# 17ai/eventql

Hardware: AMD Instinct MI355X
Metric: rows/sec scanned+aggregated, 1e9-row 4-col GROUP BY (higher is better)
Workload: dtype u64/f64; 1 GPU; config3; query=k, sum(v), count(1), sum(b) WHERE a>30000 AND b<30000 GROUP BY k, rows_per_gpu=1000000000, columns=4, encodings=UINT64_PLAIN/FLOAT_IEEE754, groups=1000, partitions=1, merge=none, groups_hint=given, float_sums=fast

## Files before the change

eventql_amd/csrc/codegen_kernels.inc:

```

namespace {

struct UpdWord {
  int word;
  int op;
  int tslot = -1;
  const char* constant = nullptr;
  bool narrow = false;
  int toff = -1;
};

struct Gen {
  const KernelPlan& kp;
  std::ostringstream s;
  const int NC, NW, S, W, SB;
  const bool grouped;
  std::vector<UpdWord> updw;

  explicit Gen(const KernelPlan& p)
      : kp(p), NC(int(p.cols.size())), NW(int(p.states.size())), S(p.lds_slots),
        W(p.words_per_slot()), SB(p.state_word_base()), grouped(p.key_mode != KEY_NONE) {
    for (const auto& a : kp.aggs) {
      switch (a.fn) {
        case EVQL_AGG_COUNT:
// ... 274 lines not shown
    for (int i = 0; i < NC; ++i) {
      if (only && !(*only)[i]) continue;
      s << ind << "u64 x" << i << "[EVQL_UNROLL][2]; u32 y" << i << "[EVQL_UNROLL][2];\n";
    }
    s << "#pragma unroll\n" << ind << "for (int u = 0; u < EVQL_UNROLL; ++u) {\n";
    s << ind << "  const u64 r = base + ((u64) (u * EVQL_BLOCK) + tid) * 2;\n";
    for (int i = 0; i < NC; ++i) {
      if (only && !(*only)[i]) continue;
      const ColAccess& c = kp.cols[i];
      switch (c.mode) {
        case ColAccess::PLAIN64:
          s << ind << "  evql_plain64_x2(A.col[" << i << "].base, A.col[" << i << "].pages, r, x" << i << "[u][0], x"
            << i << "[u][1]);\n";
          break;
        case ColAccess::PLAIN32:
          s << ind << "  evql_plain32_x2(A.col[" << i << "].base, A.col[" << i << "].pages, r, x" << i << "[u][0], x"
            << i << "[u][1]);\n";
          break;
        case ColAccess::BITPACKED:
          s << ind << "  evql_bitpacked_x2<" << c.bits << ">(A.col[" << i << "].base, A.col[" << i << "].pages, r, x"
            << i << "[u][0], x" << i << "[u][1]);\n";
          break;
        case ColAccess::NARROW:
          s << ind << "  evql_bitpacked_x2<" << c.bits << ">(A.col[" << i << "].base, r, x" << i
            << "[u][0], x" << i << "[u][1]);\n";
          break;
        case ColAccess::NARROW_F32:
          s << ind << "  evql_f32_x2(A.col[" << i << "].base, r, x" << i << "[u][0], x" << i
            << "[u][1]);\n";
          break;
        case ColAccess::SOA:
          s << ind << "  evql_soa_x2(A.col[" << i << "].soa, r, x" << i << "[u][0], x" << i
            << "[u][1]);\n";
          break;
      }
      if (c.has_tags) {
        s << ind << "  { const unsigned short tt = *reinterpret_cast<const unsigned short*>(A.col["
          << i << "].tags + r); y" << i << "[u][0] = tt & 0xffu; y" << i << "[u][1] = tt >> 8; }\n";
      } else {
        s << ind << "  y" << i << "[u][0] = 0; y" << i << "[u][1] = 0;\n";
      }
    }
    s << ind << "}\n";
  }

  bool prunes() const { return !kp.zone_conjuncts.empty(); }
  bool zone_test = false;
  template <typename Loop>
  void tile_loop_twice(const char* ind, Loop emit_loop) {
    zone_test = false;
    if (!prunes()) {
      emit_loop();
      return;
    }
    s << ind << "if (!A.tile_skip) {\n";
    emit_loop();
    s << ind << "} else {\n";
    zone_test = true;
    emit_loop();
    zone_test = false;
    s << ind << "}\n";
  }
  void zone_skip(const char* ind, const char* on_skip, bool count = true) {
    if (!zone_test) return;
    const uint64_t T = uint64_t(kp.tile_rows());
    const uint64_t zones = T >= kZoneRows ? T / kZoneRows : 1;
    s << ind << "{\n";
    if (T >= kZoneRows) {
      s << ind << "  const u64 zi = (A.tile0 + t) * " << zones << "ull;\n";
    } else {
      s << ind << "  const u64 zi = ((A.tile0 + t) * (u64) EVQL_TILE_ROWS) / EVQL_ZONE_ROWS;\n";
    }
    s << ind << "  if (evql_zones_excluded<" << zones << ">(A.tile_skip, zi)) { " << on_skip
      << (count ? " ++zskipped;" : "") << " continue; }\n";
    s << ind << "}\n";
  }
  void zone_skip_decl(const char* ind) {
    if (prunes()) s << ind << "u32 zskipped = 0;  // tiles this workgroup skipped\n";
  }
  void zone_skip_flush(const char* ind) {
    if (prunes()) s << ind << "if (tid == 0 && zskipped) atomicAdd(&A.counters[5], (u64) zskipped);\n";
  }

  void eval_call(const char* ind, int j, const std::vector<bool>* only = nullptr) {
    s << ind << "evql_eval_row(A, r + " << j << ", (r + " << j << " >= A.row_begin) && (r + " << j
      << " < A.row_end)";
    for (int i = 0; i < NC; ++i) {
      if (only && !(*only)[i]) {
        s << ", 0ull, 0u";
        continue;
      }
      s << ", x" << i << "[u][" << j << "], y" << i << "[u][" << j << "]";
    }
    s << ", o);\n";
  }

  void scan_kernel() {
    s << "struct EvqlAcc {\n  u64 passed;\n  u64 spilled;\n";
    if (!grouped) s << "  u64 w[" << (NW > 0 ? NW : 1) << "];\n";
    if (!grouped && kp.need_first_row) s << "  u64 first;\n";
    if (grouped && S > 0) {
      s << "  int cs[EVQL_LCACHE];\n  u64 cfirst[EVQL_LCACHE];\n  u64 cw[EVQL_LCACHE][EVQL_NUPD];\n"
           "  u32 cv;\n";
    }
    s << "};\n\n";
    if (grouped && S > 0) {
      s << "template <int J>\n";
      s << "__device__ __forceinline__ void evql_flush_entry(u64* lds, EvqlAcc& acc) {\n";
      s << "  const int cs = acc.cs[J];\n";
      if (kp.need_first_row) {
        s << "  evql_atomic<EVQL_OP_MIN_U64>(&" << lds_word(kp.first_row_word(), "cs") << ", acc.cfirst[J]);\n";
        s << "  acc.cfirst[J] = 0xFFFFFFFFFFFFFFFFull;\n";
      }
      for (int i = 0; i < U(); ++i) {
        s << "  evql_atomic<" << op_name(updw[i].op) << ">(&" << lds_word(SB + updw[i].word, "cs")
          << ", acc.cw[J][" << i << "]);\n";
        s << "  acc.cw[J][" << i << "] = evql_op_identity<" << op_name(updw[i].op) << ">();\n";
      }
      s << "}\n";
      s << "__device__ __forceinline__ void evql_flush_private(u64* lds, EvqlAcc& acc) {\n";
      for (int j = 0; j < kp.lane_cache; ++j) {
        s << "  if (acc.cs[" << j << "] >= 0) { evql_flush_entry<" << j << ">(lds, acc); acc.cs[" << j
          << "] = -1; }\n";
      }
      s << "}\n\n";
    }

    s << "__device__ __forceinline__ void evql_update(const EvqlArgs& A, u64* lds, EvqlAcc& acc,\n"
         "                                            const bool bypass, const u64 row, "
         "const EvqlRowOut& o) {\n";
    s << "  acc.passed += o.live ? 1 : 0;\n";
    if (!grouped) {
      if (kp.need_first_row) s << "  if (o.live && row < acc.first) acc.first = row;\n";
      for (int i = 0; i < U(); ++i) {
        s << "  if (o.uc[" << i << "]) acc.w[" << updw[i].word << "] = evql_combine<"
          << op_name(updw[i].op) << ">(acc.w[" << updw[i].word << "], o.ub[" << i << "]);\n";
      }
      s << "}\n\n";
    } else {
      auto updates = [&](bool global, const char* slot, const char* ind) {
        if (kp.need_first_row) {
          s << ind << "evql_atomic<EVQL_OP_MIN_U64>(&"
            << (global ? gtab_word(kp.first_row_word(), slot) : lds_word(kp.first_row_word(), slot))
            << ", row);\n";
        }
        for (int i = 0; i < U(); ++i) {
          s << ind << "if (o.uc[" << i << "]) evql_atomic<" << op_name(updw[i].op) << ">(&"
            << (global ? gtab_word(SB + updw[i].word, slot) : lds_word(SB + updw[i].word, slot))
            << ", o.ub[" << i << "]);\n";
        }
      };
      if (S > 0) {
        s << "  int s = -1;\n";
        s << "  if (o.live && !bypass) {\n";
        s << "    if (o.knull) { s = EVQL_LDS_SLOTS + 1; lds[s] = 0; }\n";
        s << "    else if (o.ident == EVQL_EMPTY) { s = EVQL_LDS_SLOTS; lds[s] = 0; }\n";
        if (kp.has_ident2()) {
          s << "    else s = evql_lds_find2<16>(lds, lds + EVQL_LSTRIDE, EVQL_LDS_SLOTS - 1, o.ident, "
               "o.ident2, (u32) evql_mix64(o.ident));\n";
        } else {
          s << "    else s = evql_lds_find<16>(lds, EVQL_LDS_SLOTS - 1, o.ident, (u32) "
               "evql_mix64(o.ident));\n";
        }
        s << "    if (s < 0) atomicAdd(reinterpret_cast<u32*>(&lds[EVQL_WORDS * EVQL_LSTRIDE]), 1u);\n";
        s << "  }\n";
        s << "  if (s >= 0) {\n";
        s << "    bool hit = false;\n";
        for (int j = 0; j < kp.lane_cache; ++j) {
          s << "    {\n      const bool h = acc.cs[" << j << "] == s;\n      hit = hit || h;\n";
          if (kp.need_first_row) {
            s << "      acc.cfirst[" << j << "] = (h && row < acc.cfirst[" << j << "]) ? row : acc.cfirst["
              << j << "];\n";
          }
          for (int i = 0; i < U(); ++i) {
            s << "      if (h && o.uc[" << i << "]) acc.cw[" << j << "][" << i << "] = evql_combine<"
              << op_name(updw[i].op) << ">(acc.cw[" << j << "][" << i << "], o.ub[" << i << "]);\n";
          }
          s << "    }\n";
        }
        s << "    if (!hit) {\n";
        for (int j = 0; j < kp.lane_cache; ++j) {
          s << "      {\n        const bool v = acc.cv == " << j << "u;\n";
          s << "        if (v && acc.cs[" << j << "] >= 0) evql_flush_entry<" << j << ">(lds, acc);\n";
          s << "        acc.cs[" << j << "] = v ? s : acc.cs[" << j << "];\n";
          if (kp.need_first_row) {
            s << "        acc.cfirst[" << j << "] = v ? row : acc.cfirst[" << j << "];\n";
          }
          for (int i = 0; i < U(); ++i) {
            s << "        acc.cw[" << j << "][" << i << "] = (v && o.uc[" << i << "]) ? o.ub[" << i
              << "] : acc.cw[" << j << "][" << i << "];\n";
          }
          s << "      }\n";
        }
        if (kp.lane_cache > 1) {
          s << "      acc.cv = (acc.cv + 1u) & " << (kp.lane_cache - 1) << "u;\n";
        }
        s << "    }\n  }\n";
        s << "  const bool spill = o.live && s < 0;\n";
        s << "  acc.spilled += spill ? 1 : 0;\n";
      } else {
        s << "  const bool spill = o.live;\n";
      }
      s << "  if (spill) {\n";
      s << "    i64 gs;\n";
      s << "    if (o.knull) { gs = (i64) A.gcap + 1; A.gtab[(u64) gs * EVQL_WORDS] = 0; }\n";
      s << "    else if (o.ident == EVQL_EMPTY) { gs = (i64) A.gcap; A.gtab[(u64) gs * EVQL_WORDS] = 0; }\n";
      if (kp.has_ident2()) {
        s << "    else gs = evql_gtab_find2(A.gtab, EVQL_WORDS, A.gcap, o.ident, o.ident2, "
             "evql_mix64(o.ident));\n";
      } else {
        s << "    else gs = evql_gtab_find(A.gtab, EVQL_WORDS, A.gcap, o.ident, evql_mix64(o.ident));\n";
      }
      s << "    if (gs < 0) { atomicOr(&A.status[0], EVQL_ST_TABLE_FULL); }\n";
      s << "    else {\n";
      updates(true, "gs", "      ");
      s << "    }\n  }\n}\n\n";
    }

    if (grouped && S > 0) {
      s << "__device__ __forceinline__ void evql_lds_init(u64* lds) {\n";
      s << "  if (threadIdx.x == 0) lds[EVQL_WORDS * EVQL_LSTRIDE] = 0;\n";
      s << "  for (u32 i = threadIdx.x; i < EVQL_LSTRIDE; i += blockDim.x) {\n";
      s << "    lds[i] = EVQL_EMPTY;\n";
      if (kp.has_ident2()) s << "    lds[1 * EVQL_LSTRIDE + i] = EVQL_EMPTY;\n";
      if (kp.need_first_row) {
        s << "    " << lds_word(kp.first_row_word(), "i") << " = 0xFFFFFFFFFFFFFFFFull;\n";
      }
      for (int w = 0; w < NW; ++w) {
        s << "    " << lds_word(SB + w, "i") << " = evql_op_identity<" << op_name(kp.states[w].op)
          << ">();\n";
      }
      s << "  }\n}\n\n";
      s << "template <bool EXCL>\n";
      s << "__device__ __forceinline__ void evql_lds_flush(const EvqlArgs& A, u64* lds) {\n";
      s << "  const bool excl = EXCL && evql_lds_peek32(reinterpret_cast<const u32*>(&lds[EVQL_WORDS * EVQL_LSTRIDE])) "
           "== 0;\n";
      s << "  for (u32 s = threadIdx.x; s < EVQL_LSTRIDE; s += blockDim.x) {\n";
      s << "    const u64 k = lds[s];\n    if (k == EVQL_EMPTY) continue;\n";
      s << "    i64 gs;\n";
      s << "    if (s == EVQL_LDS_SLOTS) gs = (i64) A.gcap;\n";
      s << "    else if (s == EVQL_LDS_SLOTS + 1) gs = (i64) A.gcap + 1;\n";
      if (kp.has_ident2()) {
        s << "    else gs = evql_gtab_find2(A.gtab, EVQL_WORDS, A.gcap, k, lds[EVQL_LSTRIDE + s], "
             "evql_mix64(k));\n";
      } else {
        s << "    else gs = evql_gtab_find(A.gtab, EVQL_WORDS, A.gcap, k, evql_mix64(k));\n";
      }
      s << "    if (gs < 0) { atomicOr(&A.status[0], EVQL_ST_TABLE_FULL); continue; }\n";
      s << "    if (s >= EVQL_LDS_SLOTS) A.gtab[(u64) gs * EVQL_WORDS] = 0;\n";
      s << "    if (excl) {\n";
      if (kp.need_first_row) {
        s << "      " << gtab_word(kp.first_row_word(), "gs") << " = " << lds_word(kp.first_row_word(), "s")
          << ";\n";
      }
      for (int w = 0; w < NW; ++w) {
        s << "      " << gtab_word(SB + w, "gs") << " = " << lds_word(SB + w, "s") << ";\n";
      }
      s << "      continue;\n    }\n";
      if (kp.need_first_row) {
        s << "    evql_atomic<EVQL_OP_MIN_U64>(&" << gtab_word(kp.first_row_word(), "gs") << ", "
          << lds_word(kp.first_row_word(), "s") << ");\n";
      }
      for (int w = 0; w < NW; ++w) {
        s << "    evql_atomic<" << op_name(kp.states[w].op) << ">(&" << gtab_word(SB + w, "gs") << ", "
          << lds_word(SB + w, "s") << ");\n";
      }
      s << "  }\n}\n\n";
    }

    s << "extern \"C\" __global__ void __launch_bounds__(EVQL_BLOCK) evql_scan_agg(const EvqlArgs A) {\n";
    s << "  const u32 tid = threadIdx.x;\n";
    if (grouped && S > 0) {
      s << "  __shared__ u64 lds[EVQL_WORDS * EVQL_LSTRIDE + 1];\n";
      s << "  evql_lds_init(lds);\n  __syncthreads();\n";
    } else {
      s << "  u64* lds = nullptr;\n";
    }
    s << "  EvqlAcc acc;\n  acc.passed = 0;\n  acc.spilled = 0;\n";
    if (grouped && S > 0) {
      s << "  acc.cv = 0;\n";
      for (int j = 0; j < kp.lane_cache; ++j) {
        s << "  acc.cs[" << j << "] = -1;\n  acc.cfirst[" << j << "] = 0xFFFFFFFFFFFFFFFFull;\n";
        for (int i = 0; i < U(); ++i) {
          s << "  acc.cw[" << j << "][" << i << "] = evql_op_identity<" << op_name(updw[i].op) << ">();\n";
        }
      }
    }
    if (!grouped) {
      for (int w = 0; w < NW; ++w) {
        s << "  acc.w[" << w << "] = evql_op_identity<" << op_name(kp.states[w].op) << ">();\n";
      }
      if (kp.need_first_row) s << "  acc.first = 0xFFFFFFFFFFFFFFFFull;\n";
    }
    zone_skip_decl("  ");
    tile_loop_twice("  ", [&] {
    s << "  u32 tile_no = 0;\n";
    s << "  for (u64 t = blockIdx.x; t < A.ntiles; t += gridDim.x, ++tile_no) {\n";
    zone_skip("    ", "");
    if (grouped) {
      s << "    if ((tile_no & 15u) == 0 && (__hip_atomic_load(&A.status[0], __ATOMIC_RELAXED, "
           "__HIP_MEMORY_SCOPE_AGENT) & EVQL_ST_TABLE_FULL)) break;\n";
    }
    if (grouped && S > 0) {
      s << "    const bool bypass = evql_lds_peek32(reinterpret_cast<const u32*>(&lds[EVQL_WORDS * EVQL_LSTRIDE])) "
           ">= 4u * EVQL_BLOCK;\n";
    } else {
      s << "    const bool bypass = false;\n";
    }
    s << "    const u64 base = (A.tile0 + t) * (u64) EVQL_TILE_ROWS;\n";
    tile_loads("    ");
    s << "#pragma unroll\n    for (int u = 0; u < EVQL_UNROLL; ++u) {\n";
    s << "      const u64 r = base + ((u64) (u * EVQL_BLOCK) + tid) * 2;\n";
    s << "      EvqlRowOut o;\n";
    for (int j = 0; j < 2; ++j) {
      eval_call("      ", j);
      s << "      evql_update(A, lds, acc, bypass, r + " << j << ", o);\n";
    }
    s << "    }\n  }\n";
    });

    zone_skip_flush("  ");
    s << "  {\n    const u64 p = evql_wave_reduce<EVQL_OP_ADD_U64>(acc.passed);\n";
    s << "    if ((tid & 63u) == 0 && p) atomicAdd(&A.counters[0], p);\n";
    s << "    const u64 sp = evql_wave_reduce<EVQL_OP_ADD_U64>(acc.spilled);\n";
    s << "    if ((tid & 63u) == 0 && sp) atomicAdd(&A.counters[1], sp);\n  }\n";
    if (!grouped) {
      s << "  __shared__ u64 red[(EVQL_BLOCK / 64) * " << (NW + 1) << "];\n";
      s << "  const u32 wave = tid >> 6;\n";
      for (int w = 0; w < NW; ++w) {
        s << "  { const u64 v = evql_wave_reduce<" << op_name(kp.states[w].op) << ">(acc.w[" << w
          << "]); if ((tid & 63u) == 0) red[wave * " << (NW + 1) << " + " << w << "] = v; }\n";
      }
      s << "  { const u64 v = evql_wave_reduce<EVQL_OP_ADD_U64>(acc.passed); if ((tid & 63u) == 0) "
           "red[wave * "
        << (NW + 1) << " + " << NW << "] = v; }\n";
      if (kp.need_first_row) {
        s << "  { const u64 v = evql_wave_reduce<EVQL_OP_MIN_U64>(acc.first); if ((tid & 63u) == 0 && "
             "v != 0xFFFFFFFFFFFFFFFFull) evql_atomic<EVQL_OP_MIN_U64>(&A.gtab["
          << kp.first_row_word() << "], v); }\n";
      }
      s << "  __syncthreads();\n";
      s << "  if (tid == 0) {\n";
      s << "    u64 any = 0;\n";
      s << "    for (u32 k = 0; k < EVQL_BLOCK / 64; ++k) any += red[k * " << (NW + 1) << " + " << NW
        << "];\n";
      s << "    if (any) {\n      A.gtab[0] = 0;\n";
      for (int w = 0; w < NW; ++w) {
        s << "      { u64 v = red[" << w << "]; for (u32 k = 1; k < EVQL_BLOCK / 64; ++k) v = evql_combine<"
          << op_name(kp.states[w].op) << ">(v, red[k * " << (NW + 1) << " + " << w
          << "]); evql_atomic<" << op_name(kp.states[w].op) << ">(&A.gtab[" << (SB + w)
          << "], v); }\n";
      }
      s << "    }\n  }\n";
    } else if (S > 0) {
      s << "  evql_flush_private(lds, acc);\n";
      s << "  __syncthreads();\n";
      s << "  evql_lds_flush<false>(A, lds);\n";
    }
    s << "}\n\n";
  }

  void bare_scan_kernels() {
    const int NOUT = int(kp.scan_out.size());
    std::vector<bool> where_cols(size_t(NC), false);
    if (kp.where) {
      std::vector<uint32_t> used;
      expr_inputs(kp.where, &used);
      for (uint32_t u : used) {
        if (u < uint32_t(NC)) where_cols[u] = true;
      }
    }
    int n_nullable = 0;
    for (int k = 0; k < NOUT; ++k) n_nullable += kp.scan_out_nullable[k] ? 1 : 0;
    const int stage_steps =
        uint64_t(kp.tile_rows()) * uint64_t(8 * NOUT + n_nullable) <= 48 * 1024 ? kp.unroll : 1;
    s << "#define EVQL_NOUT " << NOUT << "\n";
    s << "#define EVQL_NWAVE (EVQL_BLOCK / 64)\n";
    s << "#define EVQL_STAGE_STEPS " << stage_steps << "\n";
    s << "#define EVQL_STAGE_ROWS (EVQL_STAGE_STEPS * EVQL_BLOCK * 2)\n";
    s << "static_assert(EVQL_UNROLL * EVQL_NWAVE <= 64, \"one wave scans the wave totals of a tile\");\n";
    s << "struct EvqlScanArgs {\n"
         "  const u64* tile_offset;  // [ntiles + 1]: passing rows in front of tile t of the scan\n"
         "  u64 t0, t1;              // the window: tiles [t0, t1)\n"
         "  u64 window_base;         // tile_offset[t0]\n"
         "  u64 window_rows;         // tile_offset[t1] - window_base: rows of every output array\n"
         "  u64* words;              // [EVQL_NOUT][window_rows]\n"
         "  u8* tags;                // [EVQL_NOUT][window_rows], written for nullable outputs only\n"
         "};\n\n";
    row_function(n_literals, [&](Emitter& em) {
      s << "__device__ __forceinline__ void evql_scan_select(const EvqlArgs& A, const u64 row";
      for (int i = 0; i < NC; ++i) s << ", const u64 r" << i << ", const u32 g" << i;
      s << ", u64 (&w)[EVQL_NOUT], u32 (&q)[EVQL_NOUT]) {\n";
      col_decls();
      em.ind = "  ";
      for (int k = 0; k < NOUT; ++k) {
        const ExprPtr& e = kp.scan_out[k];
        if (e->kind == Expr::INPUT && e->type == EVQL_T_STRING) {
          s << "  w[" << k << "] = A.col[" << e->input << "].strpos[row]; q[" << k << "] = g" << e->input
            << ";\n";
          continue;
        }
        Val v = em.emit(e);
        s << em.o.str();
        em.o.str("");
        s << "  w[" << k << "] = " << Emitter::as_bits(v) << "; q[" << k << "] = " << v.g << ";\n";
      }
      s << "}\n\n";
    });
    s << "__device__ __forceinline__ void evql_run_store(u64* out, const u64 at, const u64 cap, const u64* src, "
         "u32 n) {\n"
         "  typedef u64 evql_u64x2 __attribute__((ext_vector_type(2)));\n"
         "  if (at >= cap) return;\n"
         "  if ((u64) n > cap - at) n = (u32) (cap - at);\n"
         "  u64* const dst = out + at;\n"
         "  const u32 head = (n > 0 && ((u64) dst & 8ull)) ? 1u : 0u;\n"
         "  const u32 pairs = (n - head) >> 1;\n"
         "  if (threadIdx.x == 0 && head) dst[0] = src[0];\n"
         "  for (u32 i = threadIdx.x; i < pairs; i += EVQL_BLOCK) {\n"
         "    evql_u64x2 v;\n    v.x = src[head + 2 * i];\n    v.y = src[head + 2 * i + 1];\n"
         "    *reinterpret_cast<evql_u64x2*>(dst + head + 2 * i) = v;\n  }\n"
         "  if (threadIdx.x == 0 && ((n - head) & 1u)) dst[n - 1] = src[n - 1];\n"
         "}\n\n";

    s << "extern \"C\" __global__ void __launch_bounds__(EVQL_BLOCK) evql_scan_count(const EvqlArgs A, "
         "u32* tile_count) {\n";
    s << "  const u32 tid = threadIdx.x;\n";
    s << "  __shared__ u32 wsum[EVQL_NWAVE];\n";
    zone_skip_decl("  ");
    tile_loop_twice("  ", [&] {
    s << "  for (u64 t = blockIdx.x; t < A.ntiles; t += gridDim.x) {\n";
    zone_skip("    ", "if (tid == 0) tile_count[t] = 0;");
    s << "    const u64 base = (A.tile0 + t) * (u64) EVQL_TILE_ROWS;\n";
    tile_loads("    ", &where_cols);
    s << "    u32 cnt = 0;\n";
    s << "#pragma unroll\n    for (int u = 0; u < EVQL_UNROLL; ++u) {\n";
    s << "      const u64 r = base + ((u64) (u * EVQL_BLOCK) + tid) * 2;\n";
    s << "      EvqlRowOut o;\n";
    for (int j = 0; j < 2; ++j) {
      eval_call("      ", j, &where_cols);
      s << "      cnt += (u32) __popcll(__ballot(o.live));\n";
    }
    s << "    }\n";
    s << "    if ((tid & 63u) == 0) wsum[tid >> 6] = cnt;\n";
    s << "    __syncthreads();\n";
    s << "    if (tid == 0) {\n      u32 total = 0;\n";
    s << "      for (u32 k = 0; k < EVQL_NWAVE; ++k) total += wsum[k];\n";
    s << "      tile_count[t] = total;\n    }\n";
    s << "    __syncthreads();\n";
    s << "  }\n";
    });
    zone_skip_flush("  ");
    s << "}\n\n";

    s << "extern \"C\" __global__ void __launch_bounds__(EVQL_BLOCK) evql_scan_emit(const EvqlArgs A, "
         "const EvqlScanArgs S) {\n";
    s << "  const u32 tid = threadIdx.x, lane = tid & 63u, wave = tid >> 6;\n";
    s << "  __shared__ u64 sw[EVQL_NOUT * EVQL_STAGE_ROWS];\n";
    if (n_nullable) s << "  __shared__ u8 sq[" << n_nullable << " * EVQL_STAGE_ROWS];\n";
    s << "  __shared__ u32 wpre[EVQL_UNROLL * EVQL_NWAVE + 1];\n";
    s << "  for (u64 t = S.t0 + blockIdx.x; t < S.t1; t += gridDim.x) {\n";
    s << "    const u64 dst0 = S.tile_offset[t] - S.window_base;\n";
    s << "    if (S.tile_offset[t + 1] == S.tile_offset[t]) continue;\n";
    s << "    const u64 base = (A.tile0 + t) * (u64) EVQL_TILE_ROWS;\n";
    tile_loads("    ");
    s << "    u32 live = 0;  // bit 2u + j: row (u, j) of this lane passes\n";
    s << "#pragma unroll\n    for (int u = 0; u < EVQL_UNROLL; ++u) {\n";
    s << "      const u64 r = base + ((u64) (u * EVQL_BLOCK) + tid) * 2;\n";
    s << "      EvqlRowOut o;\n";
    s << "      u32 wcnt = 0;\n";
    for (int j = 0; j < 2; ++j) {
      eval_call("      ", j);
      s << "      live |= o.live ? (1u << (2 * u + " << j << ")) : 0u;\n";
      s << "      wcnt += (u32) __popcll(__ballot(o.live));\n";
    }
    s << "      if (lane == 0) wpre[u * EVQL_NWAVE + wave] = wcnt;\n";
    s << "    }\n    __syncthreads();\n";
    s << "    if (wave == 0) {\n";
    s << "      const u32 v = lane < EVQL_UNROLL * EVQL_NWAVE ? wpre[lane] : 0u;\n";
    s << "      u32 incl = v;\n";
    s << "#pragma unroll\n      for (int d = 1; d < 64; d <<= 1) { const u32 x = __shfl_up(incl, d, 64); "
         "if ((int) lane >= d) incl += x; }\n";
    s << "      if (lane < EVQL_UNROLL * EVQL_NWAVE) wpre[lane] = incl - v;\n";
    s << "      if (lane == EVQL_UNROLL * EVQL_NWAVE - 1) wpre[EVQL_UNROLL * EVQL_NWAVE] = incl;\n";
    s << "    }\n    __syncthreads();\n";
    s << "#pragma unroll\n    for (int u0 = 0; u0 < EVQL_UNROLL; u0 += EVQL_STAGE_STEPS) {\n";
    s << "      const u32 g0 = wpre[u0 * EVQL_NWAVE], g1 = wpre[(u0 + EVQL_STAGE_STEPS) * EVQL_NWAVE];\n";
    s << "#pragma unroll\n      for (int u = u0; u < u0 + EVQL_STAGE_STEPS; ++u) {\n";
    s << "        const u64 r = base + ((u64) (u * EVQL_BLOCK) + tid) * 2;\n";
    s << "        const bool l0 = (live >> (2 * u)) & 1u, l1 = (live >> (2 * u + 1)) & 1u;\n";
    s << "        const u64 b0 = __ballot(l0), b1 = __ballot(l1);\n";
    s << "        u32 rank = wpre[u * EVQL_NWAVE + wave] - g0;\n";
    s << "        rank = __builtin_amdgcn_mbcnt_hi((u32) (b0 >> 32), __builtin_amdgcn_mbcnt_lo((u32) b0, rank));\n";
    s << "        rank = __builtin_amdgcn_mbcnt_hi((u32) (b1 >> 32), __builtin_amdgcn_mbcnt_lo((u32) b1, rank));\n";
    for (int j = 0; j < 2; ++j) {
      s << "        if (l" << j << ") {\n";
      s << "          u64 w[EVQL_NOUT]; u32 q[EVQL_NOUT];\n";
      s << "          evql_scan_select(A, r + " << j;
      for (int i = 0; i < NC; ++i) s << ", x" << i << "[u][" << j << "], y" << i << "[u][" << j << "]";
      s << ", w, q);\n";
      int nk = 0;
      for (int k = 0; k < NOUT; ++k) {
        s << "          sw[" << k << " * EVQL_STAGE_ROWS + rank] = w[" << k << "];\n";
        if (kp.scan_out_nullable[k]) {
          s << "          sq[" << nk++ << " * EVQL_STAGE_ROWS + rank] = (u8) (q[" << k << "] & 1u);\n";
        }
      }
      s << "          rank += 1;\n        }\n";
    }
    s << "      }\n      __syncthreads();\n";
    s << "      const u32 n = g1 - g0;\n";
    s << "      const u64 at = dst0 + g0;\n";
    {
      int nk = 0;
      for (int k = 0; k < NOUT; ++k) {
        s << "      evql_run_store(S.words + " << k << " * S.window_rows, at, S.window_rows, sw + " << k
          << " * EVQL_STAGE_ROWS, n);\n";
        if (kp.scan_out_nullable[k]) {
          s << "      for (u32 i = tid; i < n && at + i < S.window_rows; i += EVQL_BLOCK) S.tags[" << k
            << " * S.window_rows + at + i] = sq[" << nk++ << " * EVQL_STAGE_ROWS + i];\n";
        }
      }
    }
    s << "      __syncthreads();\n";
    s << "    }\n  }\n}\n\n";
  }

  void where_rows_kernel() {
    s << "extern \"C\" __global__ void __launch_bounds__(EVQL_BLOCK) evql_where_rows(const EvqlArgs A, "
         "u8* acc) {\n";
    s << "  const u32 tid = threadIdx.x;\n";
    s << "  for (u64 t = blockIdx.x; t < A.ntiles; t += gridDim.x) {\n";
    s << "    const u64 base = (A.tile0 + t) * (u64) EVQL_TILE_ROWS;\n";
    tile_loads("    ");
    s << "#pragma unroll\n    for (int u = 0; u < EVQL_UNROLL; ++u) {\n";
    s << "      const u64 r = base + ((u64) (u * EVQL_BLOCK) + tid) * 2;\n";
    s << "      EvqlRowOut o;\n";
    for (int j = 0; j < 2; ++j) {
      eval_call("      ", j);
      s << "      if (r + " << j << " < A.row_end) acc[r + " << j << "] = o.live ? 1 : 0;\n";
    }
    s << "    }\n  }\n}\n\n";
  }

  void partition_kernels() {
    const int frw = kp.first_row_word();
    s << "#define EVQL_PBITS " << kp.part_bits << "\n#define EVQL_NPART " << (1 << kp.part_bits)
      << "\n";
    s << "__device__ __forceinline__ u32 evql_bucket(u64 ident) { return (u32) (evql_mix64(ident ^ "
         "0x5851f42d4c957f2dull) >> (64 - EVQL_PBITS)); }\n\n";
    const int cbits = kp.part_bits <= 8 ? kp.part_bits : 6;
    const int fbits = kp.part_bits - cbits;
    s << "#define EVQL_CBITS " << cbits << "\n#define EVQL_FBITS " << fbits << "\n";
    s << "#define EVQL_NCOARSE " << (1 << cbits) << "\n#define EVQL_NFINE " << (1 << fbits) << "\n";
    s << "struct EvqlPartArgs {\n  u64 tiles_per_wg;\n  u32* counts;      // [bucket][workgroup]\n"
         "  const u64* bucket_start;  // [NPART + 1] tuple index\n  u64* tuples;\n  u64 nwg;\n"
         "  u64* tuples_tmp;  // coarse-bucket order (two-level only)\n"
         "  u32* cursors;     // [NCOARSE] + [NPART] reservation cursors, zeroed per launch\n"
         "  u64* dense;       // dense group records [kind, identity, ...] of the buckets\n"
         "  u64 dense_cap;    // ... whose groups all fitted the LDS table (records)\n"
         "  u64 coarse_cap;   // fused form: capacity (tuples) of every coarse bucket of tuples_tmp\n};\n\n";
    const bool fused = kp.part_fused && fbits > 0;
    s << "#define EVQL_ST_PART_OVERFLOW 64u\n";
    if (fused) {
      s << "#define EVQL_CSTART(c_) ((u64) (c_) * P.coarse_cap)\n";
      s << "#define EVQL_CEND(c_) ((u64) (c_) * P.coarse_cap + ((u64) P.cursors[c_] < P.coarse_cap ? "
           "(u64) P.cursors[c_] : P.coarse_cap))\n";
    } else {
      s << "#define EVQL_CSTART(c_) (P.bucket_start[(u64) (c_) << EVQL_FBITS])\n";
      s << "#define EVQL_CEND(c_) (P.bucket_start[(u64) ((c_) + 1) << EVQL_FBITS])\n";
    }
    s << "__device__ __forceinline__ void evql_tuple_store(u32* p, const u32* v) {\n"
         "#pragma unroll\n"
         "  for (int x = 0; x < EVQL_TUPLE_U32; x += (EVQL_TUPLE_U32 % 4 == 0 ? 4 : 2)) {\n"
         "    if (EVQL_TUPLE_U32 % 4 == 0) *reinterpret_cast<uint4*>(p + x) = make_uint4(v[x], v[x + 1], "
         "v[x + 2], v[x + 3]);\n"
         "    else *reinterpret_cast<uint2*>(p + x) = make_uint2(v[x], v[x + 1]);\n  }\n}\n";
    s << "__device__ __forceinline__ void evql_tuple_load(const u32* p, u32* v) {\n"
         "#pragma unroll\n"
         "  for (int x = 0; x < EVQL_TUPLE_U32; x += (EVQL_TUPLE_U32 % 4 == 0 ? 4 : 2)) {\n"
         "    if (EVQL_TUPLE_U32 % 4 == 0) { const uint4 t = *reinterpret_cast<const uint4*>(p + x); "
         "v[x] = t.x; v[x + 1] = t.y; v[x + 2] = t.z; v[x + 3] = t.w; }\n"
         "    else { const uint2 t = *reinterpret_cast<const uint2*>(p + x); v[x] = t.x; v[x + 1] = "
         "t.y; }\n  }\n}\n\n";

    if (!fused) {
    s << "extern \"C\" __global__ void __launch_bounds__(EVQL_BLOCK) evql_part_count(const EvqlArgs A, "
         "const EvqlPartArgs P) {\n";
    s << "  const u32 tid = threadIdx.x;\n";
    s << "  __shared__ u32 hist[EVQL_NPART];\n";
    s << "  for (u32 i = tid; i < EVQL_NPART; i += EVQL_BLOCK) hist[i] = 0;\n  __syncthreads();\n";
    s << "  const u64 t0 = (u64) blockIdx.x * P.tiles_per_wg;\n";
    s << "  const u64 t1 = t0 + P.tiles_per_wg < A.ntiles ? t0 + P.tiles_per_wg : A.ntiles;\n";
    tile_loop_twice("  ", [&] {
    s << "  for (u64 t = t0; t < t1; ++t) {\n";
    zone_skip("    ", "", false);
    s << "    const u64 base = (A.tile0 + t) * (u64) EVQL_TILE_ROWS;\n";
    tile_loads("    ");
    s << "#pragma unroll\n    for (int u = 0; u < EVQL_UNROLL; ++u) {\n";
    s << "      const u64 r = base + ((u64) (u * EVQL_BLOCK) + tid) * 2;\n";
    s << "      EvqlRowOut o;\n";
    for (int j = 0; j < 2; ++j) {
      eval_call("      ", j);
      s << "      if (o.live) atomicAdd(&hist[evql_bucket(o.ident)], 1u);\n";
    }
    s << "    }\n  }\n";
    });
    s << "  __syncthreads();\n";
    s << "  for (u32 i = tid; i < EVQL_NPART; i += EVQL_BLOCK) P.counts[(u64) i * P.nwg + blockIdx.x] = "
         "hist[i];\n";
    s << "}\n\n";
    }

    s << "extern \"C\" __global__ void __launch_bounds__(EVQL_BLOCK) evql_part_scatter(const EvqlArgs A, "
         "const EvqlPartArgs P) {\n";
    s << "  const u32 tid = threadIdx.x;\n";
    s << "  __shared__ u32 hist[EVQL_NCOARSE];\n";
    s << "  __shared__ u64 gbase[EVQL_NCOARSE];\n";
    if (fused) {
      s << "  __shared__ u32 fhist[EVQL_NPART];\n";
      s << "  for (u32 i = tid; i < EVQL_NPART; i += EVQL_BLOCK) fhist[i] = 0;\n";
    }
    s << "  u32* const dst = reinterpret_cast<u32*>(EVQL_FBITS ? P.tuples_tmp : P.tuples);\n";
    s << "  u64 passed = 0;\n";
    s << "  const u64 t0 = (u64) blockIdx.x * P.tiles_per_wg;\n";
    s << "  const u64 t1 = t0 + P.tiles_per_wg < A.ntiles ? t0 + P.tiles_per_wg : A.ntiles;\n";
    zone_skip_decl("  ");
    tile_loop_twice("  ", [&] {
    s << "  for (u64 t = t0; t < t1; ++t) {\n";
    zone_skip("    ", "");
    s << "    const u64 base = (A.tile0 + t) * (u64) EVQL_TILE_ROWS;\n";
    tile_loads("    ");
    s << "    for (u32 i = tid; i < EVQL_NCOARSE; i += EVQL_BLOCK) hist[i] = 0;\n";
    s << "    __syncthreads();\n";
    s << "#pragma unroll\n    for (int u = 0; u < EVQL_UNROLL; ++u) {\n";
    s << "      const u64 r = base + ((u64) (u * EVQL_BLOCK) + tid) * 2;\n";
    s << "      EvqlRowOut o;\n";
    for (int j = 0; j < 2; ++j) {
      eval_call("      ", j);
      s << "      if (o.live) atomicAdd(&hist[evql_bucket(o.ident) >> EVQL_FBITS], 1u);\n";
    }
    s << "    }\n    __syncthreads();\n";
    s << "    for (u32 i = tid; i < EVQL_NCOARSE; i += EVQL_BLOCK) {\n";
    s << "      const u32 c = hist[i];\n";
    if (fused) {
      s << "      u64 gb = EVQL_EMPTY;\n";
      s << "      if (c) {\n";
      s << "        const u64 at = (u64) atomicAdd(&P.cursors[i], c);\n";
      s << "        if (at + c <= P.coarse_cap) gb = (u64) i * P.coarse_cap + at;\n";
      s << "        else atomicOr(&A.status[0], EVQL_ST_PART_OVERFLOW);\n";
      s << "      }\n";
      s << "      gbase[i] = gb;\n";
    } else {
      s << "      gbase[i] = P.bucket_start[(u64) i << EVQL_FBITS] + (c ? (u64) atomicAdd(&P.cursors[i], c) "
           ": 0ull);\n";
    }
    s << "      hist[i] = 0;\n    }\n    __syncthreads();\n";
    s << "#pragma unroll\n    for (int u = 0; u < EVQL_UNROLL; ++u) {\n";
    s << "      const u64 r = base + ((u64) (u * EVQL_BLOCK) + tid) * 2;\n";
    s << "      EvqlRowOut o;\n";
    for (int j = 0; j < 2; ++j) {
      eval_call("      ", j);
      s << "      if (o.live) {\n";
      s << "        passed += 1;\n";
      if (fused) {
        s << "        const u32 fb = evql_bucket(o.ident);\n";
        s << "        const u32 b = fb >> EVQL_FBITS;\n";
        s << "        atomicAdd(&fhist[fb], 1u);\n";
      } else {
        s << "        const u32 b = evql_bucket(o.ident) >> EVQL_FBITS;\n";
      }
      s << "        const u64 pos = gbase[b] + atomicAdd(&hist[b], 1u);\n";
      s << "        u32 tv[EVQL_TUPLE_U32];\n";
      s << "        tv[EVQL_TUPLE_U32 - 1] = 0;\n";
      tuple_put("        ", off_ident, kp.narrow_ident, "o.ident");
      if (kp.has_ident2()) tuple_put("        ", off_ident2, false, "o.ident2");
      if (kp.need_first_row) {
        tuple_put("        ", off_row, kp.narrow_first_row, "r + " + std::to_string(j));
      }
      for (int i = 0; i < U(); ++i) {
        if (updw[i].tslot < 0) continue;
        tuple_put("        ", updw[i].toff, updw[i].narrow, "o.ub[" + std::to_string(i) + "]");
      }
      if (fused) {
        s << "        if (gbase[b] != EVQL_EMPTY) evql_tuple_store(dst + pos * EVQL_TUPLE_U32, tv);\n";
      } else {
        s << "        evql_tuple_store(dst + pos * EVQL_TUPLE_U32, tv);\n";
      }
      s << "      }\n";
    }
    s << "    }\n    __syncthreads();\n  }\n";
    });
    if (fused) {
      s << "  __syncthreads();\n";
      s << "  for (u32 i = tid; i < EVQL_NPART; i += EVQL_BLOCK) {\n";
      s << "    const u32 c = fhist[i];\n";
      s << "    if (c) atomicAdd(const_cast<u64*>(&P.bucket_start[i]), (u64) c);\n  }\n";
    }
    zone_skip_flush("  ");
    s << "  { const u64 p = evql_wave_reduce<EVQL_OP_ADD_U64>(passed);\n";
    s << "    if ((tid & 63u) == 0 && p) atomicAdd(&A.counters[0], p); }\n";
    s << "}\n\n";

    if (fbits > 0) {
      const int TWn = tuple_u32;
      const int rtif = TWn <= 4 ? 4 : (TWn <= 8 ? 2 : 1);
      s << "#define EVQL_RTIF " << rtif << "\n";
      s << "extern \"C\" __global__ void __launch_bounds__(EVQL_BLOCK) evql_part_refine(const EvqlArgs "
           "A, const EvqlPartArgs P) {\n";
      s << "  const u32 tid = threadIdx.x;\n";
      if (fused) {
        s << "  if (__hip_atomic_load(&A.status[0], __ATOMIC_RELAXED, __HIP_MEMORY_SCOPE_AGENT) & "
             "EVQL_ST_PART_OVERFLOW) return;\n";
      }
// ... 211 lines not shown
```

eventql_amd/csrc/evql_device.h:

```cpp
#ifndef EVQL_DEVICE_H
#define EVQL_DEVICE_H

typedef unsigned long long u64;
typedef long long i64;
typedef unsigned int u32;
typedef unsigned char u8;

#define EVQL_EMPTY 0xFFFFFFFFFFFFFFFFull
#define EVQL_MAX_COLS 16
#define EVQL_MAX_LITS 32
#define EVQL_WAVE 64

#define EVQL_ST_DIV_BY_ZERO 1u
#define EVQL_ST_TABLE_FULL 2u
#define EVQL_ST_MOD_BY_ZERO 4u

struct EvqlColArg {
  const u64* pages;
  const u64* soa;
  const u8* tags;
  u64 npages;
  const u64* strpos;
  const u8* base;
};
// ... 243 lines not shown
  return true;
}
__device__ __forceinline__ bool evql_str_affix(const EvqlStr& s, const EvqlStr& affix, bool at_end) {
  if (s.len < affix.len) return false;
  const u32 off = at_end ? s.len - affix.len : 0;
  for (u32 i = 0; i < affix.len; ++i) {
    if (evql_str_byte(s, off + i) != evql_str_byte(affix, i)) return false;
  }
  return true;
}
__device__ __forceinline__ int evql_str_cmp(const EvqlStr& a, const EvqlStr& b) {
  const u32 n = a.len < b.len ? a.len : b.len;
  for (u32 i = 0; i < n; ++i) {
    const u32 x = evql_str_byte(a, i), y = evql_str_byte(b, i);
    if (x != y) return x < y ? -1 : 1;
    if (x == 0) break;
  }
  return a.len < b.len ? -1 : (a.len > b.len ? 1 : 0);
}

__device__ __forceinline__ double evql_as_f64(u64 v) { return __longlong_as_double((i64) v); }
__device__ __forceinline__ u64 evql_f64_bits(double v) { return (u64) __double_as_longlong(v); }

#define EVQL_OP_ADD_U64 0
#define EVQL_OP_ADD_F64 1
#define EVQL_OP_MIN_U64 2
#define EVQL_OP_MAX_U64 3
#define EVQL_OP_MIN_I64 4
#define EVQL_OP_MAX_I64 5
#define EVQL_OP_MIN_F64 6
#define EVQL_OP_MAX_F64 7

template <int OP>
__device__ __forceinline__ u64 evql_op_identity() {
  switch (OP) {
    case EVQL_OP_MIN_U64: return 0xFFFFFFFFFFFFFFFFull;
    case EVQL_OP_MAX_U64: return 0ull;
    case EVQL_OP_MIN_I64: return 0x7FFFFFFFFFFFFFFFull;
    case EVQL_OP_MAX_I64: return 0x8000000000000000ull;
    case EVQL_OP_MIN_F64: return 0x7FF0000000000000ull;
    case EVQL_OP_MAX_F64: return 0xFFF0000000000000ull;
    default: return 0ull;
  }
}

template <int OP>
__device__ __forceinline__ u64 evql_combine(u64 a, u64 b) {
  switch (OP) {
    case EVQL_OP_ADD_U64: return a + b;
    case EVQL_OP_ADD_F64: return evql_f64_bits(evql_as_f64(a) + evql_as_f64(b));
    case EVQL_OP_MIN_U64: return a < b ? a : b;
    case EVQL_OP_MAX_U64: return a > b ? a : b;
    case EVQL_OP_MIN_I64: return (i64) a < (i64) b ? a : b;
    case EVQL_OP_MAX_I64: return (i64) a > (i64) b ? a : b;
    case EVQL_OP_MIN_F64: return evql_as_f64(b) < evql_as_f64(a) ? b : a;
    case EVQL_OP_MAX_F64: return evql_as_f64(b) > evql_as_f64(a) ? b : a;
  }
  return a;
}

template <int OP>
__device__ __forceinline__ void evql_atomic(u64* p, u64 v) {
  switch (OP) {
    case EVQL_OP_ADD_U64: atomicAdd(p, v); break;
    case EVQL_OP_ADD_F64: unsafeAtomicAdd(reinterpret_cast<double*>(p), evql_as_f64(v)); break;
    case EVQL_OP_MIN_U64: atomicMin(p, v); break;
    case EVQL_OP_MAX_U64: atomicMax(p, v); break;
    case EVQL_OP_MIN_I64: atomicMin(reinterpret_cast<i64*>(p), (i64) v); break;
    case EVQL_OP_MAX_I64: atomicMax(reinterpret_cast<i64*>(p), (i64) v); break;
    case EVQL_OP_MIN_F64: unsafeAtomicMin(reinterpret_cast<double*>(p), evql_as_f64(v)); break;
    case EVQL_OP_MAX_F64: unsafeAtomicMax(reinterpret_cast<double*>(p), evql_as_f64(v)); break;
  }
}


__device__ __forceinline__ u64 evql_lds_peek(const u64* p) {
  return __hip_atomic_load(p, __ATOMIC_RELAXED, __HIP_MEMORY_SCOPE_WORKGROUP);
}
__device__ __forceinline__ u32 evql_lds_peek32(const u32* p) {
  return __hip_atomic_load(p, __ATOMIC_RELAXED, __HIP_MEMORY_SCOPE_WORKGROUP);
}

template <int MAXP>
__device__ __forceinline__ int evql_lds_find(u64* keys, u32 mask, u64 ident, u32 h) {
  u32 s = (u32) ident & mask;
  {
    u64 cur = evql_lds_peek(&keys[s]);
    if (cur == ident) return (int) s;
    if (cur == EVQL_EMPTY) {
      u64 old = atomicCAS(&keys[s], EVQL_EMPTY, ident);
      if (old == EVQL_EMPTY || old == ident) return (int) s;
    }
  }
  s = h & mask;
#pragma unroll 1
  for (int probe = 0; probe < MAXP; ++probe) {
    u64 cur = evql_lds_peek(&keys[s]);
    if (cur == ident) return (int) s;
    if (cur == EVQL_EMPTY) {
      u64 old = atomicCAS(&keys[s], EVQL_EMPTY, ident);
      if (old == EVQL_EMPTY || old == ident) return (int) s;
    }
    s = (s + 1) & mask;
  }
  return -1;
}

#define EVQL_GTAB_MAX_PROBE 128
__device__ __forceinline__ i64 evql_gtab_find(u64* tab, u32 W, u64 cap, u64 ident, u64 h) {
  const u64 mask = cap - 1;
  u64 s = h & mask;
  const u64 maxp = cap < EVQL_GTAB_MAX_PROBE ? cap : EVQL_GTAB_MAX_PROBE;
#pragma unroll 1
  for (u64 probe = 0; probe < maxp; ++probe) {
    u64* key = tab + s * W;
    u64 cur = __hip_atomic_load(key, __ATOMIC_RELAXED, __HIP_MEMORY_SCOPE_AGENT);
    if (cur == ident) return (i64) s;
    if (cur == EVQL_EMPTY) {
      u64 old = atomicCAS(key, EVQL_EMPTY, ident);
      if (old == EVQL_EMPTY || old == ident) return (i64) s;
    }
    s = (s + 1) & mask;
  }
  return -1;
}

template <int MAXP>
__device__ __forceinline__ int evql_lds_find2(u64* keys, u64* keys2, u32 mask, u64 ident,
                                              u64 ident2, u32 h) {
  u32 s = (u32) ident & mask;
#pragma unroll 1
  for (int probe = 0; probe <= MAXP; ++probe) {
    u64 cur = evql_lds_peek(&keys[s]);
    if (cur == EVQL_EMPTY) cur = atomicCAS(&keys[s], EVQL_EMPTY, ident);
    if (cur == EVQL_EMPTY || cur == ident) {
      u64 c2 = evql_lds_peek(&keys2[s]);
      if (c2 == EVQL_EMPTY) c2 = atomicCAS(&keys2[s], EVQL_EMPTY, ident2);
      if (c2 == EVQL_EMPTY || c2 == ident2) return (int) s;
    }
    s = probe == 0 ? (h & mask) : ((s + 1) & mask);
  }
  return -1;
}

__device__ __forceinline__ i64 evql_gtab_find2(u64* tab, u32 W, u64 cap, u64 ident, u64 ident2,
                                               u64 h) {
  const u64 mask = cap - 1;
  u64 s = h & mask;
  const u64 maxp = cap < EVQL_GTAB_MAX_PROBE ? cap : EVQL_GTAB_MAX_PROBE;
#pragma unroll 1
  for (u64 probe = 0; probe < maxp; ++probe) {
    u64* key = tab + s * W;
    u64 cur = __hip_atomic_load(key, __ATOMIC_RELAXED, __HIP_MEMORY_SCOPE_AGENT);
    if (cur == EVQL_EMPTY) cur = atomicCAS(key, EVQL_EMPTY, ident);
    if (cur == EVQL_EMPTY || cur == ident) {
      u64 c2 = __hip_atomic_load(key + 1, __ATOMIC_RELAXED, __HIP_MEMORY_SCOPE_AGENT);
      if (c2 == EVQL_EMPTY) c2 = atomicCAS(key + 1, EVQL_EMPTY, ident2);
      if (c2 == EVQL_EMPTY || c2 == ident2) return (i64) s;
    }
    s = (s + 1) & mask;
  }
  return -1;
}

#define EVQL_ST_PAIRSET_FULL 8u
__device__ __forceinline__ u64 evql_pairset_insert(const EvqlArgs& A, int which, u64 ident,
                                                   u64 value, u64 flags, bool spare_flag_bits) {
  u64* tab = A.pairset[which];
  const u64 cap = A.pairset_cap[which];
  const u64 mask = cap - 1;
  if (ident == EVQL_EMPTY) {
    ident = EVQL_EMPTY - 1;
    flags = spare_flag_bits ? (flags | 2u) : (flags ^ 0x9e3779b97f4a7c15ull);
  }
  if (value == EVQL_EMPTY) {
    value = EVQL_EMPTY - 1;
    flags = spare_flag_bits ? (flags | 4u) : (flags ^ 0xc2b2ae3d27d4eb4full);
  }
  if (flags == EVQL_EMPTY) flags = EVQL_EMPTY - 1;
  u64 s = evql_mix64(evql_hash_combine(evql_hash_combine(ident, value), flags)) & mask;
  const u64 maxp = cap < 256 ? cap : 256;
#pragma unroll 1
  for (u64 probe = 0; probe < maxp; ++probe, s = (s + 1) & mask) {
    u64 c0 = __hip_atomic_load(tab + s, __ATOMIC_RELAXED, __HIP_MEMORY_SCOPE_AGENT);
    if (c0 == EVQL_EMPTY) c0 = atomicCAS(tab + s, EVQL_EMPTY, ident);
    if (c0 != EVQL_EMPTY && c0 != ident) continue;
    u64 c1 = __hip_atomic_load(tab + cap + s, __ATOMIC_RELAXED, __HIP_MEMORY_SCOPE_AGENT);
    if (c1 == EVQL_EMPTY) c1 = atomicCAS(tab + cap + s, EVQL_EMPTY, value);
// ... 28 lines not shown
```

Before: 461.9 billion rows/s.

## Batch LDS probe peeks across row pairs and use 32-bit row window checks

```diff
diff --git a/eventql_amd/csrc/codegen_kernels.inc b/eventql_amd/csrc/codegen_kernels.inc
--- a/eventql_amd/csrc/codegen_kernels.inc
+++ b/eventql_amd/csrc/codegen_kernels.inc
@@ -380,9 +380,25 @@
     if (prunes()) s << ind << "if (tid == 0 && zskipped) atomicAdd(&A.counters[5], (u64) zskipped);\n";
   }
 
-  void eval_call(const char* ind, int j, const std::vector<bool>* only = nullptr) {
-    s << ind << "evql_eval_row(A, r + " << j << ", (r + " << j << " >= A.row_begin) && (r + " << j
-      << " < A.row_end)";
+  bool window32 = true;
+  void tile_window(const char* ind) {
+    if (!window32) return;
+    s << ind << "const u64 wb = A.row_begin > base ? A.row_begin - base : 0ull;\n";
+    s << ind << "const u64 we = A.row_end > base ? A.row_end - base : 0ull;\n";
+    s << ind << "const u32 wlo = (u32) (wb < (u64) EVQL_TILE_ROWS ? wb : (u64) EVQL_TILE_ROWS);\n";
+    s << ind << "const u32 whi = (u32) (we < (u64) EVQL_TILE_ROWS ? we : (u64) EVQL_TILE_ROWS);\n";
+    s << ind << "const u32 wlen = whi > wlo ? whi - wlo : 0u;\n";
+    s << ind << "const u32 wrel = 2u * tid - wlo;\n";
+  }
+  void eval_call(const char* ind, int j, const std::vector<bool>* only = nullptr,
+                 const char* out = "o") {
+    if (window32) {
+      s << ind << "evql_eval_row(A, r + " << j << ", wrel + (u32) (u * EVQL_BLOCK * 2 + " << j
+        << ") < wlen";
+    } else {
+      s << ind << "evql_eval_row(A, r + " << j << ", (r + " << j << " >= A.row_begin) && (r + " << j
+        << " < A.row_end)";
+    }
     for (int i = 0; i < NC; ++i) {
       if (only && !(*only)[i]) {
         s << ", 0ull, 0u";
@@ -390,9 +406,10 @@
       }
       s << ", x" << i << "[u][" << j << "], y" << i << "[u][" << j << "]";
     }
-    s << ", o);\n";
-  }
-
+    s << ", " << out << ");\n";
+  }
+
+  bool probe_ahead() const { return grouped && S > 0 && !kp.has_ident2(); }
   void scan_kernel() {
     s << "struct EvqlAcc {\n  u64 passed;\n  u64 spilled;\n";
     if (!grouped) s << "  u64 w[" << (NW > 0 ? NW : 1) << "];\n";
@@ -426,7 +443,8 @@
 
     s << "__device__ __forceinline__ void evql_update(const EvqlArgs& A, u64* lds, EvqlAcc& acc,\n"
          "                                            const bool bypass, const u64 row, "
-         "const EvqlRowOut& o) {\n";
+         "const EvqlRowOut& o"
+      << (probe_ahead() ? ", const u64 slot0" : "") << ") {\n";
     s << "  acc.passed += o.live ? 1 : 0;\n";
     if (!grouped) {
       if (kp.need_first_row) s << "  if (o.live && row < acc.first) acc.first = row;\n";
@@ -457,43 +475,62 @@
           s << "    else s = evql_lds_find2<16>(lds, lds + EVQL_LSTRIDE, EVQL_LDS_SLOTS - 1, o.ident, "
                "o.ident2, (u32) evql_mix64(o.ident));\n";
         } else {
-          s << "    else s = evql_lds_find<16>(lds, EVQL_LDS_SLOTS - 1, o.ident, (u32) "
-               "evql_mix64(o.ident));\n";
+          s << "    else s = evql_lds_find" << (probe_ahead() ? "_from" : "")
+            << "<16>(lds, EVQL_LDS_SLOTS - 1, o.ident, (u32) evql_mix64(o.ident)"
+            << (probe_ahead() ? ", slot0" : "") << ");\n";
         }
         s << "    if (s < 0) atomicAdd(reinterpret_cast<u32*>(&lds[EVQL_WORDS * EVQL_LSTRIDE]), 1u);\n";
         s << "  }\n";
-        s << "  if (s >= 0) {\n";
-        s << "    bool hit = false;\n";
-        for (int j = 0; j < kp.lane_cache; ++j) {
-          s << "    {\n      const bool h = acc.cs[" << j << "] == s;\n      hit = hit || h;\n";
-          if (kp.need_first_row) {
-            s << "      acc.cfirst[" << j << "] = (h && row < acc.cfirst[" << j << "]) ? row : acc.cfirst["
-              << j << "];\n";
+        if (kp.lane_cache == 1) {
+          s << "  const bool hit = s >= 0 && acc.cs[0] == s;\n";
+          s << "  const bool miss = s >= 0 && !hit;\n";
+          s << "  if (hit) {\n    asm volatile(\"\");\n";
+          if (kp.need_first_row) s << "    if (row < acc.cfirst[0]) acc.cfirst[0] = row;\n";
+          for (int i = 0; i < U(); ++i) {
+            s << "    if (o.uc[" << i << "]) acc.cw[0][" << i << "] = evql_combine<" << op_name(updw[i].op)
+              << ">(acc.cw[0][" << i << "], o.ub[" << i << "]);\n";
           }
-          for (int i = 0; i < U(); ++i) {
-            s << "      if (h && o.uc[" << i << "]) acc.cw[" << j << "][" << i << "] = evql_combine<"
-              << op_name(updw[i].op) << ">(acc.cw[" << j << "][" << i << "], o.ub[" << i << "]);\n";
+          s << "  }\n";
+          s << "  if (miss) {\n";
+          s << "    if (acc.cs[0] >= 0) evql_flush_entry<0>(lds, acc);\n";
+          s << "    acc.cs[0] = s;\n";
+          if (kp.need_first_row) s << "    acc.cfirst[0] = row;\n";
+          for (int i = 0; i < U(); ++i) s << "    acc.cw[0][" << i << "] = o.ub[" << i << "];\n";
+          s << "  }\n";
+        } else {
+          s << "  if (s >= 0) {\n";
+          s << "    bool hit = false;\n";
+          for (int j = 0; j < kp.lane_cache; ++j) {
+            s << "    {\n      const bool h = acc.cs[" << j << "] == s;\n      hit = hit || h;\n";
+            if (kp.need_first_row) {
+              s << "      acc.cfirst[" << j << "] = (h && row < acc.cfirst[" << j << "]) ? row : acc.cfirst["
+                << j << "];\n";
+            }
+            for (int i = 0; i < U(); ++i) {
+              s << "      if (h && o.uc[" << i << "]) acc.cw[" << j << "][" << i << "] = evql_combine<"
+                << op_name(updw[i].op) << ">(acc.cw[" << j << "][" << i << "], o.ub[" << i << "]);\n";
+            }
+            s << "    }\n";
           }
-          s << "    }\n";
+          s << "    if (!hit) {\n";
+          for (int j = 0; j < kp.lane_cache; ++j) {
+            s << "      {\n        const bool v = acc.cv == " << j << "u;\n";
+            s << "        if (v && acc.cs[" << j << "] >= 0) evql_flush_entry<" << j << ">(lds, acc);\n";
+            s << "        acc.cs[" << j << "] = v ? s : acc.cs[" << j << "];\n";
+            if (kp.need_first_row) {
+              s << "        acc.cfirst[" << j << "] = v ? row : acc.cfirst[" << j << "];\n";
+            }
+            for (int i = 0; i < U(); ++i) {
+              s << "        acc.cw[" << j << "][" << i << "] = (v && o.uc[" << i << "]) ? o.ub[" << i
+                << "] : acc.cw[" << j << "][" << i << "];\n";
+            }
+            s << "      }\n";
+          }
+          if (kp.lane_cache > 1) {
+            s << "      acc.cv = (acc.cv + 1u) & " << (kp.lane_cache - 1) << "u;\n";
+          }
+          s << "    }\n  }\n";
         }
-        s << "    if (!hit) {\n";
-        for (int j = 0; j < kp.lane_cache; ++j) {
-          s << "      {\n        const bool v = acc.cv == " << j << "u;\n";
-          s << "        if (v && acc.cs[" << j << "] >= 0) evql_flush_entry<" << j << ">(lds, acc);\n";
-          s << "        acc.cs[" << j << "] = v ? s : acc.cs[" << j << "];\n";
-          if (kp.need_first_row) {
-            s << "        acc.cfirst[" << j << "] = v ? row : acc.cfirst[" << j << "];\n";
-          }
-          for (int i = 0; i < U(); ++i) {
-            s << "        acc.cw[" << j << "][" << i << "] = (v && o.uc[" << i << "]) ? o.ub[" << i
-              << "] : acc.cw[" << j << "][" << i << "];\n";
-          }
-          s << "      }\n";
-        }
-        if (kp.lane_cache > 1) {
-          s << "      acc.cv = (acc.cv + 1u) & " << (kp.lane_cache - 1) << "u;\n";
-        }
-        s << "    }\n  }\n";
         s << "  const bool spill = o.live && s < 0;\n";
         s << "  acc.spilled += spill ? 1 : 0;\n";
       } else {
@@ -591,6 +628,7 @@
       if (kp.need_first_row) s << "  acc.first = 0xFFFFFFFFFFFFFFFFull;\n";
     }
     zone_skip_decl("  ");
+    window32 = grouped;
     tile_loop_twice("  ", [&] {
     s << "  u32 tile_no = 0;\n";
     s << "  for (u64 t = blockIdx.x; t < A.ntiles; t += gridDim.x, ++tile_no) {\n";
@@ -606,16 +644,30 @@
       s << "    const bool bypass = false;\n";
     }
     s << "    const u64 base = (A.tile0 + t) * (u64) EVQL_TILE_ROWS;\n";
+    tile_window("    ");
     tile_loads("    ");
     s << "#pragma unroll\n    for (int u = 0; u < EVQL_UNROLL; ++u) {\n";
     s << "      const u64 r = base + ((u64) (u * EVQL_BLOCK) + tid) * 2;\n";
-    s << "      EvqlRowOut o;\n";
-    for (int j = 0; j < 2; ++j) {
-      eval_call("      ", j);
-      s << "      evql_update(A, lds, acc, bypass, r + " << j << ", o);\n";
+    if (probe_ahead()) {
+      s << "      EvqlRowOut o0, o1;\n";
+      for (int j = 0; j < 2; ++j) eval_call("      ", j, nullptr, j ? "o1" : "o0");
+      for (int j = 0; j < 2; ++j) {
+        s << "      const u64 k" << j << " = evql_lds_peek(&lds[(u32) o" << j
+          << ".ident & (EVQL_LDS_SLOTS - 1)]);\n";
+      }
+      for (int j = 0; j < 2; ++j) {
+        s << "      evql_update(A, lds, acc, bypass, r + " << j << ", o" << j << ", k" << j << ");\n";
+      }
+    } else {
+      s << "      EvqlRowOut o;\n";
+      for (int j = 0; j < 2; ++j) {
+        eval_call("      ", j);
+        s << "      evql_update(A, lds, acc, bypass, r + " << j << ", o);\n";
+      }
     }
     s << "    }\n  }\n";
     });
+    window32 = true;
 
     zone_skip_flush("  ");
     s << "  {\n    const u64 p = evql_wave_reduce<EVQL_OP_ADD_U64>(acc.passed);\n";
@@ -725,10 +777,12 @@
     s << "  const u32 tid = threadIdx.x;\n";
     s << "  __shared__ u32 wsum[EVQL_NWAVE];\n";
     zone_skip_decl("  ");
+    window32 = false;
     tile_loop_twice("  ", [&] {
     s << "  for (u64 t = blockIdx.x; t < A.ntiles; t += gridDim.x) {\n";
     zone_skip("    ", "if (tid == 0) tile_count[t] = 0;");
     s << "    const u64 base = (A.tile0 + t) * (u64) EVQL_TILE_ROWS;\n";
+    tile_window("    ");
     tile_loads("    ", &where_cols);
     s << "    u32 cnt = 0;\n";
     s << "#pragma unroll\n    for (int u = 0; u < EVQL_UNROLL; ++u) {\n";
@@ -747,6 +801,7 @@
     s << "    __syncthreads();\n";
     s << "  }\n";
     });
+    window32 = true;
     zone_skip_flush("  ");
     s << "}\n\n";
 
@@ -760,6 +815,7 @@
     s << "    const u64 dst0 = S.tile_offset[t] - S.window_base;\n";
     s << "    if (S.tile_offset[t + 1] == S.tile_offset[t]) continue;\n";
     s << "    const u64 base = (A.tile0 + t) * (u64) EVQL_TILE_ROWS;\n";
+    tile_window("    ");
     tile_loads("    ");
     s << "    u32 live = 0;  // bit 2u + j: row (u, j) of this lane passes\n";
     s << "#pragma unroll\n    for (int u = 0; u < EVQL_UNROLL; ++u) {\n";
@@ -829,6 +885,7 @@
     s << "  const u32 tid = threadIdx.x;\n";
     s << "  for (u64 t = blockIdx.x; t < A.ntiles; t += gridDim.x) {\n";
     s << "    const u64 base = (A.tile0 + t) * (u64) EVQL_TILE_ROWS;\n";
+    tile_window("    ");
     tile_loads("    ");
     s << "#pragma unroll\n    for (int u = 0; u < EVQL_UNROLL; ++u) {\n";
     s << "      const u64 r = base + ((u64) (u * EVQL_BLOCK) + tid) * 2;\n";
@@ -889,10 +946,12 @@
     s << "  for (u32 i = tid; i < EVQL_NPART; i += EVQL_BLOCK) hist[i] = 0;\n  __syncthreads();\n";
     s << "  const u64 t0 = (u64) blockIdx.x * P.tiles_per_wg;\n";
     s << "  const u64 t1 = t0 + P.tiles_per_wg < A.ntiles ? t0 + P.tiles_per_wg : A.ntiles;\n";
+    window32 = false;
     tile_loop_twice("  ", [&] {
     s << "  for (u64 t = t0; t < t1; ++t) {\n";
     zone_skip("    ", "", false);
     s << "    const u64 base = (A.tile0 + t) * (u64) EVQL_TILE_ROWS;\n";
+    tile_window("    ");
     tile_loads("    ");
     s << "#pragma unroll\n    for (int u = 0; u < EVQL_UNROLL; ++u) {\n";
     s << "      const u64 r = base + ((u64) (u * EVQL_BLOCK) + tid) * 2;\n";
@@ -903,6 +962,7 @@
     }
     s << "    }\n  }\n";
     });
+    window32 = true;
     s << "  __syncthreads();\n";
     s << "  for (u32 i = tid; i < EVQL_NPART; i += EVQL_BLOCK) P.counts[(u64) i * P.nwg + blockIdx.x] = "
          "hist[i];\n";
@@ -927,6 +987,7 @@
     s << "  for (u64 t = t0; t < t1; ++t) {\n";
     zone_skip("    ", "");
     s << "    const u64 base = (A.tile0 + t) * (u64) EVQL_TILE_ROWS;\n";
+    tile_window("    ");
     tile_loads("    ");
     s << "    for (u32 i = tid; i < EVQL_NCOARSE; i += EVQL_BLOCK) hist[i] = 0;\n";
     s << "    __syncthreads();\n";
diff --git a/eventql_amd/csrc/evql_device.h b/eventql_amd/csrc/evql_device.h
--- a/eventql_amd/csrc/evql_device.h
+++ b/eventql_amd/csrc/evql_device.h
@@ -349,10 +349,9 @@
 }
 
 template <int MAXP>
-__device__ __forceinline__ int evql_lds_find(u64* keys, u32 mask, u64 ident, u32 h) {
+__device__ __forceinline__ int evql_lds_find_from(u64* keys, u32 mask, u64 ident, u32 h, u64 cur) {
   u32 s = (u32) ident & mask;
   {
-    u64 cur = evql_lds_peek(&keys[s]);
     if (cur == ident) return (int) s;
     if (cur == EVQL_EMPTY) {
       u64 old = atomicCAS(&keys[s], EVQL_EMPTY, ident);
@@ -371,6 +370,10 @@
     s = (s + 1) & mask;
   }
   return -1;
+}
+template <int MAXP>
+__device__ __forceinline__ int evql_lds_find(u64* keys, u32 mask, u64 ident, u32 h) {
+  return evql_lds_find_from<MAXP>(keys, mask, ident, h, evql_lds_peek(&keys[(u32) ident & mask]));
 }
 
 #define EVQL_GTAB_MAX_PROBE 128
```

Result: faster. 505.2 billion rows/s, median of 6 (+9.4%).
